# YujiaoShi/HighlyAccurate

Hardware: AMD Instinct MI355X
Metric: image-pairs/sec through N-iter LM pose loop, KITTI shapes (higher is better)
Workload: dtype bf16; 1 GPU; BASELINE configs[1]: LM_S2GP.forward(mode='test'), sat 512x512, grd 256x1024, VGG-16 two-branch, level 3, 5 LM iters x 3 levels, 3-DoF, random-init weights; pairs_per_gpu=32, global_batch=32, parallelism=batch-sharded x1, no collective

## Files before the change

### highlyaccurate_amd/csrc/common.h

```cpp
#pragma once
#include <hip/hip_runtime.h>
#include <atomic>
#include <stdarg.h>
#include <stdio.h>
#include "../../include/hla.h"

void hla_set_error(const char* fmt, ...);

enum { K_PACK = 0, K_CONV02, K_CONV_NT2, K_CONV_NT2_POOL, K_CONV_NT1, K_CONV_NT1_POOL, K_CONF, K_L2NORM,
       K_LM256, K_LM128, K_LM64, K_LM16, K_LMSOLVE, K_GRIDSAMPLE, K_LMBWD, K_WGRAD, K_ELEMWISE, K_LMREPAIR };
void hla_prof_begin(int id, double flops, double bytes, hipStream_t st);
void hla_prof_begin_dyn(int id, double flops, double bytes, hipStream_t st, const int* dev_live, int denom);
void hla_prof_end(hipStream_t st);
bool hla_prof_on();

#ifndef HLA_CONV_STAMPS
#define HLA_CONV_STAMPS 0
#endif
#if HLA_CONV_STAMPS
constexpr int HLA_STAMP_N = 8;
struct HlaStampCfg { unsigned long long* buf; int want; int counter; unsigned grid_x, grid_y; };
extern HlaStampCfg g_hla_stamp;
#endif

#define HLA_CHECK_HIP(expr)                                                              \
  do {                                                                                   \
    hipError_t _e = (expr);                                                              \
    if (_e != hipSuccess) {                                                              \
      hla_set_error("%s failed: %s (%s:%d)", #expr, hipGetErrorString(_e), __FILE__, __LINE__); \
      return HLA_ERR_HIP;                                                                \
    }                                                                                    \
  } while (0)

static inline bool hla_dtype_ok(int dtype) { return dtype == HLA_F32 || dtype == HLA_BF16 || dtype == HLA_F16 || dtype == HLA_F16X3; }

struct split32;
template <typename T> struct HlaType { using type = T; };
template <typename F> static inline auto hla_dispatch_dtype(int dtype, F&& f) {
  if (dtype == HLA_BF16) return f(HlaType<__bf16>{});
  if (dtype == HLA_F16) return f(HlaType<_Float16>{});
  if (dtype == HLA_F16X3) return f(HlaType<split32>{});
  return f(HlaType<float>{});
}

#define HLA_REQUIRE(cond, ...)      \
  do {                              \
    if (!(cond)) {                  \
      hla_set_error(__VA_ARGS__);   \
      return HLA_ERR_ARG;           \
    }                               \
  } while (0)

struct HlaPerDeviceOnce {
// ... 25 lines not shown
```

### highlyaccurate_amd/csrc/conv_kernels.h

```cpp
#pragma once
#include "common.h"
#include "conv_block_map.h"
#include <type_traits>

typedef __bf16 bf16;
typedef _Float16 f16;
using f32x16 = __attribute__((ext_vector_type(16))) float;
using bf16x8 = __attribute__((ext_vector_type(8))) __bf16;
using f16x8 = __attribute__((ext_vector_type(8))) _Float16;
using f16x4 = __attribute__((ext_vector_type(4))) _Float16;

struct split32 {
  float v;
  split32() = default;
  __host__ __device__ explicit split32(float f) : v(f) {}
  __host__ __device__ explicit operator float() const { return v; }
};
template <typename T> struct Prec { static constexpr bool SPLIT = false; static constexpr int CEPL = 16 / (int)sizeof(T); };
template <> struct Prec<split32> { static constexpr bool SPLIT = true; static constexpr int CEPL = 8; };

__device__ __host__ __forceinline__ float split_scale(unsigned amax_bits) {
  int E = (int)(amax_bits >> 23) & 0xff;
  E = E < 81 ? 81 : (E > 201 ? 201 : E);
  const unsigned bits = (unsigned)(127 + 141 - E) << 23;
// ... 166 lines not shown
  size_t wg0_x_plane;
  float* wg0_part;
#if HLA_CONV_STAMPS
  unsigned long long* stamps;
#endif
};
template <int NT> __host__ __device__ __forceinline__ int conv_cout_blocks(const ConvArgs& a) { return NT == 1 ? 1 : a.Cout / (64 * NT); }
#if HLA_CONV_STAMPS
#define HLA_STAMP(K) do { if (a.stamps) { const unsigned long long ts_ = __builtin_readcyclecounter(); \
    if ((threadIdx.x & 63) == 0) a.stamps[((size_t)blockIdx.x * 4 +(threadIdx.x >> 6)) * HLA_STAMP_N + (K)] = ts_; } } while (0)
#define HLA_STAMP_HWID() do { if (a.stamps && (threadIdx.x & 63) == 0) { \
    const unsigned long long hw_ = __builtin_amdgcn_s_getreg((31 << 11) | (0 << 6) | 4), xc_ = __builtin_amdgcn_s_getreg((31 << 11) | (0 << 6) | 20); \
    a.stamps[((size_t)blockIdx.x * 4 +(threadIdx.x >> 6)) * HLA_STAMP_N + 7] = hw_ | (xc_ << 32); } } while (0)
#else
#define HLA_STAMP(K) do {} while (0)
#define HLA_STAMP_HWID() do {} while (0)
#endif

struct ConvDyn {
  int n_live;
  int list;
  int src_bands;
  int add_bands;
};
struct PixBox { int y0, y1, x0, x1; };

constexpr int HWID = 34;
constexpr int SB = 64;
constexpr int PSTR = 64;
__device__ __forceinline__ int halo_key(int hx) { return (hx >> 2) & 3; }
__device__ __forceinline__ int halo_off(int pix, int hx, int slot) { return pix * PSTR + ((slot ^ halo_key(hx)) << 4); }
constexpr int HALO_TAP0 = 2, HALO_TAP1 = 6;
constexpr int HLA_CONV_DMA_TAP = 1;
struct FragOff { int o[3][2]; };
template <int SHAPE = SHAPE_32x32x16>
__device__ __forceinline__ FragOff frag_offsets(int lane, int row0) {
  FragOff f;
  if constexpr (SHAPE == SHAPE_16x16x32) {
    const int x = lane & 15, slot = lane >> 4;
#pragma unroll
    for (int kx = 0; kx < 3; ++kx)
#pragma unroll
      for (int p = 0; p < 2; ++p) f.o[kx][p] = halo_off(row0 * HWID + 16 * p + x + kx, 16 * p + x + kx, slot);
  } else {
    const int x = lane & 31, g = lane >> 5;
#pragma unroll
    for (int kx = 0; kx < 3; ++kx)
#pragma unroll
      for (int kg = 0; kg < 2; ++kg) f.o[kx][kg] = halo_off(row0 * HWID + x + kx, x + kx, g | (kg << 1));
  }
  return f;
}

__device__ __forceinline__ float lane_xor1(float v) {
  return __int_as_float(__builtin_amdgcn_update_dpp(0, __float_as_int(v), 0xB1, 0xF, 0xF, false));
}

template <typename E, int NT> struct RowStager {
  static constexpr int CW = NT * 32, PITCH = CW * (int)sizeof(E) + 16, CPP = CW * (int)sizeof(E) / 16;
  static __device__ __forceinline__ void put(char* stage, int px, int ch, float v0, float v1, float v2, float v3) {
    store4((E*)(stage + px * PITCH) + ch, v0, v1, v2, v3);
  }
  template <bool PLAIN = false, int GG = 2>
  static __device__ __forceinline__ float flush(const char* stage, E* dst, int npx, int npx_valid, int Cout, int lane,
                                                const E* mask = nullptr, const E* add = nullptr,
                                                int add_px_lo = 0, int add_px_hi = 1 << 30) {
// ... 450 lines not shown
        } else {
          const uint4 A = frag_kmajor<ET>(stage, PITCH, kk * KPX, 0, lane);
          ET e[EPV];
#pragma unroll
          for (int jj = 0; jj < EPV; ++jj) {
            const int k = sizeof(ET) == 2 ? 8 * g5 + jj : 2 * jj + g5;
            e[jj] = (ET)(j < 27 ? row[k] : (j == 27 ? 1.f : 0.f));
          }
          mma16<ET>(accw, A, __builtin_bit_cast(uint4, e));
        }
      }
      if (SPLIT) {
        const float ds = j == 27 ? 1.f / sG : 1.f / (sG * s_in);
#pragma unroll
        for (int r = 0; r < 16; ++r) accw[r] += tmp[r] * ds;
      }
    }
  }
  if (wm == 1) {
#pragma unroll
    for (int r = 0; r < 16; ++r) xr[(wn * 16 + r) * 64 + lane] = accw[r];
  }
  __syncthreads();
  if (wm == 0) {
    float* dst = a.wg0_part + (size_t)blockIdx.x * 64 * 32;
#pragma unroll
    for (int r = 0; r < 16; ++r) {
      const int co = cb + (r & 3) + 8 * (r >> 2) + 4 * g5;
      dst[co * 32 + j] = accw[r] + xr[(wn * 16 + r) * 64 + lane];
    }
  }
}

template <typename T, int MT, int NT, int WD, int PF = (NT == 1 ? 4 : 3)>
struct WeightRing {
  static constexpr int RS = WD + 1;
  uint4 wb[RS][2][NT];
  static constexpr int PFD = PF;
  uint4 pf[PFD + 1];
  const uint4* wq[NT];

  __device__ __forceinline__ void prime() {
#pragma unroll
    for (int d = 0; d < WD; ++d)
#pragma unroll
      for (int kg = 0; kg < 2; ++kg)
#pragma unroll
        for (int j = 0; j < NT; ++j) wb[d][kg][j] = wq[j][(d * 2 + kg) * 64];
  }
  __device__ __forceinline__ void next_stage() {
#pragma unroll
    for (int j = 0; j < NT; ++j) wq[j] += 18 * 64;
    if (9 % RS != 0) {
      uint4 tmp[WD][2][NT];
#pragma unroll
      for (int d = 0; d < WD; ++d)
#pragma unroll
        for (int kg = 0; kg < 2; ++kg)
#pragma unroll
          for (int j = 0; j < NT; ++j) tmp[d][kg][j] = wb[(9 + d) % RS][kg][j];
#pragma unroll
      for (int d = 0; d < WD; ++d)
#pragma unroll
        for (int kg = 0; kg < 2; ++kg)
#pragma unroll
          for (int j = 0; j < NT; ++j) wb[d][kg][j] = tmp[d][kg][j];
    }
  }
};

__device__ __forceinline__ void stagger_priority() {
  const unsigned slot = __builtin_amdgcn_s_getreg((3 << 11) | (0 << 6) | 4);
  if (slot & 1) __builtin_amdgcn_s_setprio(1);
}

template <typename T, int MT, int NT, int WD, int PF, int SHAPE = SHAPE_32x32x16, typename Mid>
__device__ __forceinline__ void stage_mma(typename AccMap<SHAPE>::Tile (&acc)[MT][NT], const char* cur, const FragOff& fo,
                                          WeightRing<T, MT, NT, WD, PF>& ring, Mid&& mid) {
  constexpr int RS = WD + 1;
#pragma unroll
  for (int tap = 0; tap < 9; ++tap) {
#pragma unroll
    for (int kg = 0; kg < 2; ++kg)
#pragma unroll
      for (int j = 0; j < NT; ++j) ring.wb[(tap + WD) % RS][kg][j] = ring.wq[j][((tap + WD) * 2 + kg) * 64];
    mid(tap);
    constexpr int FPT = MT * 2, DEPTH = PF;
    auto frag_ptr = [&](int f) {
      const int tp = tap + f / FPT, r = f % FPT;
      return cur + fo.o[tp % 3][r & 1] + (tp / 3 + (r >> 1)) * HWID * PSTR;
    };
    if (tap == 0) {
#pragma unroll
      for (int f = 0; f < DEPTH; ++f) ring.pf[f] = *(const uint4*)frag_ptr(f);
    }
    __builtin_amdgcn_sched_barrier(0);
#pragma unroll
    for (int f = 0; f < FPT; ++f) {
      const int slot = (tap * FPT + f) % (DEPTH + 1), nslot = (tap * FPT + f + DEPTH) % (DEPTH + 1);
      if (tap * FPT + f + DEPTH < 9 * FPT) ring.pf[nslot] = *(const uint4*)frag_ptr(f + DEPTH);
      const int i = f >> 1, kg = f & 1;
      if constexpr (Prec<T>::SPLIT) {
#pragma unroll
        for (int c = 0; c < (kg == 0 ? 2 : 1); ++c)
#pragma unroll
          for (int j = 0; j < NT; ++j) mma16<T>(acc[i][j], ring.wb[tap % RS][c][j], ring.pf[slot]);
      } else if constexpr (SHAPE == SHAPE_16x16x32) {
#pragma unroll
        for (int c = 0; c < 2; ++c)
#pragma unroll
          for (int j = 0; j < NT; ++j) mma32<T>(acc[i][j].t[2 * kg + c], ring.wb[tap % RS][c][j], ring.pf[slot]);
      } else {
#pragma unroll
        for (int j = 0; j < NT; ++j) mma16<T>(acc[i][j], ring.wb[tap % RS][kg][j], ring.pf[slot]);
      }
      __builtin_amdgcn_sched_barrier(0);
    }
  }
  ring.next_stage();
}

template <typename T, int MT, int NT, int WM, bool UNPOOL = false>
constexpr int conv3x3_lds_bytes() {
  constexpr int HP = (WM * MT + 2) * HWID, NP = (HP * 4 + 255) / 256;
  constexpr int buf = ((sizeof(T) == 2 && !UNPOOL && !Prec<T>::SPLIT) ? NP * 64 : HP) * PSTR;
  constexpr int stg = 32 * (RowStager<float, NT>::PITCH + (sizeof(T) == 2 ? RowStager<T, NT>::PITCH : 0));
  return 2 * buf > 4 * stg ? 2 * buf : 4 * stg;
}
template <typename T, int MT, int NT, int WM, int WN, bool POOL, int WD, bool UNPOOL = false, int SHAPE = SHAPE_32x32x16, bool XLDS = false>
__device__ __forceinline__ void conv3x3_body(const ConvArgs& a, const int blk, const int nblk) {
  static_assert(WM * WN == 4, "4 waves per block");
  static_assert(SHAPE == SHAPE_32x32x16 || (sizeof(T) == 2 && !UNPOOL), "16x16x32: bf16 / f16 forward kernels only");
  using M = AccMap<SHAPE>;
  constexpr int EPL = 16 / sizeof(T), KC = SB / sizeof(T);
  constexpr int TH = WM * MT, HPIX = (TH + 2) * HWID;
  constexpr int NPIECE = (HPIX * 4 + 255) / 256;
  constexpr bool DMA = sizeof(T) == 2 && !UNPOOL && !Prec<T>::SPLIT;
  constexpr int BUF = (DMA ? NPIECE * 64 : HPIX) * PSTR;
  constexpr int NHALF = (NPIECE + 1) / 2;
  constexpr int STG = 32 * (RowStager<float, NT>::PITCH + (sizeof(T) == 2 ? RowStager<T, NT>::PITCH : 0));
  constexpr int LDSB = 2 * BUF > 4 * STG ? 2 * BUF : 4 * STG;
  static_assert(LDSB == conv3x3_lds_bytes<T, MT, NT, WM, UNPOOL>(), "conv3x3_lds_bytes is what a launch with XLDS allocates");
  __shared__ __attribute__((aligned(16))) char lds_own[XLDS ? 16 : LDSB];
  extern __shared__ __attribute__((aligned(16))) char lds_dyn[];
  char* const lds = XLDS ? lds_dyn : lds_own;
  __shared__ float red[8];

  HLA_STAMP(0);
  HLA_STAMP_HWID();
  const int t = threadIdx.x, lane = t & 63, wv = __builtin_amdgcn_readfirstlane(t >> 6), wm = wv / WN, wn = wv % WN;
  const int sy0 = a.src_row_lo, sy1 = a.H;
  int tx, ty, b, cblk;
  const int gy = conv_cout_blocks<NT>(a);
  const int clo = a.col_begin * 32;
  struct { int lo0, lo1, lo2, hi0, hi1, hi2; } sb = {clo, clo, clo, a.W, a.W, a.W};
  if (a.dyn) {
    const ConvDyn& d = *(const ConvDyn*)(a.dyn + a.dyn_desc);
    const int nl = d.n_live, nlive = nl * a.B;
    if (blk >= nlive * gy) return;
    const ConvBlock m = conv_block_map(blk, nlive * gy, gy);
    const int bid = m.tile;
    cblk = __builtin_amdgcn_readfirstlane(m.cb);
    b = bid / nl;
    const int e = a.dyn[d.list + bid % nl];
// ... 142 lines not shown
                   HLA_DMA_LD(4, 7, 8) HLA_DMA_STEP HLA_DMA_LD(5, 7, 8) HLA_DMA_STEP HLA_DMA_LD(6, 7, 8) "s_mov_b32 m0, %0"             \
                   : "=&s"(keep) : "v"(O[0]), "v"(O[1]), "v"(O[2]), "v"(O[3]), "v"(O[4]), "v"(O[5]), "s"(rs), "s"(soff), "s"(dst)      \
                   : "memory", "scc")
      if (first) HLA_DMA6(off1); else HLA_DMA6(off2);
#undef HLA_DMA6
    } else if constexpr (NPIECE == 4) {
#define HLA_DMA4(O)                                                                                                                    \
      asm volatile(HLA_DMA_HEAD(7) HLA_DMA_LD(1, 5, 6) HLA_DMA_STEP HLA_DMA_LD(2, 5, 6) HLA_DMA_STEP HLA_DMA_LD(3, 5, 6) HLA_DMA_STEP    \
                   HLA_DMA_LD(4, 5, 6) "s_mov_b32 m0, %0"                                                                              \
                   : "=&s"(keep) : "v"(O[0]), "v"(O[1]), "v"(O[2]), "v"(O[3]), "s"(rs), "s"(soff), "s"(dst) : "memory", "scc")
      if (first) HLA_DMA4(off1); else HLA_DMA4(off2);
#undef HLA_DMA4
    }
#undef HLA_DMA_HEAD
#undef HLA_DMA_LD
#undef HLA_DMA_STEP
  };

  const int ntg0 = (cblk * WN + wn) * NT;
  typename M::Tile acc[MT][NT];
#pragma unroll
  for (int j = 0; j < NT; ++j)
#pragma unroll
    for (int q = 0; q < 4; ++q) {
      float4 b4 = make_float4(0.f, 0.f, 0.f, 0.f);
      if (sizeof(T) == 2 && a.bias) b4 = *(const float4*)(a.bias + (ntg0 + j) * 32 + M::ch(lane, q));
#pragma unroll
      for (int i = 0; i < MT; ++i) {
        M::set(acc[i][j], q, 0, b4.x); M::set(acc[i][j], q, 1, b4.y); M::set(acc[i][j], q, 2, b4.z); M::set(acc[i][j], q, 3, b4.w);
      }
    }

  const FragOff fo = frag_offsets<SHAPE>(lane, wm * MT);
  constexpr int PF = NT == 1 ? (UNPOOL && sizeof(T) == 2 ? 3 : 4) : 3;
  WeightRing<T, MT, NT, WD, PF> ring;
#pragma unroll
  for (int j = 0; j < NT; ++j) ring.wq[j] = a.wpk + (size_t)(ntg0 + j) * nstage * 18 * 64 + lane;

  uint4 st[NHALF];
  StageIds ids;
  ring.prime();
  if constexpr (DMA) {
    dma_stage(0, 0);
    asm volatile("s_waitcnt vmcnt(0)" ::: "memory");
  } else {
    uint4 st1[NHALF];
    StageIds ids1;
    load_stage(0, 0, st, ids);
    load_stage(0, 1, st1, ids1);
    write_stage(lds, 0, 0, st, ids);
    write_stage(lds, 0, 1, st1, ids1);
  }
  __syncthreads();
  HLA_STAMP(1);
  stagger_priority();

  for (int sg = 0; sg < nstage; ++sg) {
    const bool more = sg + 1 < nstage;
    char* nxt = lds + ((sg + 1) & 1) * BUF;
    stage_mma<T, MT, NT, WD, PF, SHAPE>(acc, lds + (sg & 1) * BUF, fo, ring, [&](int tap) __attribute__((always_inline)) {
      if constexpr (DMA) {
        if (tap == HLA_CONV_DMA_TAP && more) dma_stage(sg + 1, (sg + 1) & 1);
      } else {
        if (tap == HALO_TAP0 && more) load_stage(sg + 1, 0, st, ids);
        if (tap == HALO_TAP1 && more) { write_stage(nxt, sg + 1, 0, st, ids); load_stage(sg + 1, 1, st, ids); }
      }
    });
    if constexpr (DMA) {
      static_assert(!DMA || HLA_CONV_DMA_TAP <= 8 - WD, "the halo DMA must be issued before the next stage's weight fragments");
      if (more) asm volatile("s_waitcnt vmcnt(%0)" ::"n"(2 * NT * WD) : "memory");
    } else {
      if (more) write_stage(nxt, sg + 1, 1, st, ids);
    }
    if (sg == 0) HLA_STAMP(2);
    __syncthreads();
    if (sg == 0) HLA_STAMP(3);
  }
  HLA_STAMP(4);
  static_assert((LDSB / 4) % 16 == 0, "stager alignment");
  {
    char* stager = lds + wv * (LDSB / 4);
    const int mode = epilogue_mode(a);
    PixBox addb{a.add_row_lo, 1 << 30, 0, 1 << 30};
    if (a.dyn) {
      const ConvDyn& d = *(const ConvDyn*)(a.dyn + a.dyn_desc);
      if (d.add_bands >= 0) {
        const int band = (POOL ? y0 >> 1 : y0) >> 3;
        addb.x0 = a.dyn[d.add_bands + 2 * band];
        addb.x1 = a.dyn[d.add_bands + 2 * band + 1];
      }
    }
    constexpr bool RAW_SPECIAL = POOL || NT == 1;
    constexpr bool T16 = sizeof(T) == 2;
    if constexpr (UNPOOL && NT == 1 && MT == 4 && WN == 2) {
      if (mode == EPI_DGRAD_WG0) {
        conv_epilogue_wg0<T, MT>(acc, a, b, y0, x0, lds, dsc);
        HLA_STAMP(5);
        return;
      }
    }
    if (mode == EPI_ACT) conv_epilogue<T, MT, NT, POOL, EPI_ACT, false, LDSB / 4, SHAPE>(acc, a, b, y0 + wm * MT, x0, ntg0 * 32, red, stager, dsc, addb, nullptr, blk, nblk);
    else if (T16 && RAW_SPECIAL && a.raw16 && mode == EPI_ACT_RAW)
      conv_epilogue<T, MT, NT, POOL, (T16 && RAW_SPECIAL) ? EPI_ACT_RAW : EPI_GENERIC, T16 && RAW_SPECIAL, 0, SHAPE>(acc, a, b, y0 + wm * MT, x0, ntg0 * 32, red, stager, dsc, addb, nullptr, blk, nblk);
    else if (T16 && a.raw16 && mode == EPI_ACT_RAW_NOBIAS)
      conv_epilogue<T, MT, NT, POOL, T16 ? EPI_ACT_RAW_NOBIAS : EPI_GENERIC, T16, 0, SHAPE>(acc, a, b, y0 + wm * MT, x0, ntg0 * 32, red, stager, dsc, addb, nullptr, blk, nblk);
    else if (RAW_SPECIAL && mode == EPI_ACT_RAW) conv_epilogue<T, MT, NT, POOL, RAW_SPECIAL ? EPI_ACT_RAW : EPI_GENERIC, false, 0, SHAPE>(acc, a, b, y0 + wm * MT, x0, ntg0 * 32, red, stager, dsc, addb, nullptr, blk, nblk);
    else if (SHAPE == SHAPE_32x32x16 && mode == EPI_DGRAD)
      conv_epilogue<T, MT, NT, POOL, SHAPE == SHAPE_32x32x16 ? EPI_DGRAD : EPI_GENERIC, false, 0, SHAPE>(acc, a, b, y0 + wm * MT, x0, ntg0 * 32, red, stager, dsc, addb, nullptr, blk, nblk);
    else if ((RAW_SPECIAL || sizeof(T) == 2) && mode == EPI_ACT_RAW_NOBIAS)
      conv_epilogue<T, MT, NT, POOL, (RAW_SPECIAL || sizeof(T) == 2) ? EPI_ACT_RAW_NOBIAS : EPI_GENERIC, false, 0, SHAPE>(acc, a, b, y0 + wm * MT, x0, ntg0 * 32, red, stager, dsc, addb, nullptr, blk, nblk);
    else conv_epilogue<T, MT, NT, POOL, EPI_GENERIC, false, 0, SHAPE>(acc, a, b, y0 + wm * MT, x0, ntg0 * 32, red, stager, dsc, addb, nullptr, blk, nblk);
  }
  HLA_STAMP(5);
}
template <typename T, int MT, int NT, int WM, int WN, bool POOL, int WD, bool UNPOOL = false, int SHAPE = SHAPE_32x32x16>
__global__ __launch_bounds__(256, NT == 1 ? 3 : 2) void conv3x3_kernel(ConvArgs a) {
  conv3x3_body<T, MT, NT, WM, WN, POOL, WD, UNPOOL, SHAPE>(a, (int)blockIdx.x, (int)gridDim.x);
}

template <typename A> struct PairArgs { A s[2]; int n0; };
template <typename A>
__device__ __forceinline__ A kernarg_block(unsigned word_off) {
  static_assert(sizeof(A) % 4 == 0, "argument blocks are fetched as 32-bit words");
  typedef const __attribute__((address_space(4))) unsigned* kptr_t;
  const kptr_t kp = (kptr_t)__builtin_amdgcn_kernarg_segment_ptr() + word_off;
  unsigned w[sizeof(A) / 4];
#pragma unroll
  for (unsigned i = 0; i < sizeof(A) / 4; ++i) w[i] = kp[i];
  A a;
  __builtin_memcpy(&a, w, sizeof(A));
  return a;
}
template <typename A>
__device__ __forceinline__ A pair_segment_args(bool second) {
  static_assert(offsetof(PairArgs<A>, s) == 0, "the argument blocks lead the kernarg segment");
  return kernarg_block<A>(second ? sizeof(A) / 4 : 0);
}
template <typename P> __device__ __forceinline__ P* pair_global(P* p) {
  return (P*)(__attribute__((address_space(1))) P*)(unsigned long long)p;
}
__device__ __forceinline__ void pair_inference_args(ConvArgs& a) {
  a.src1 = pair_global(a.src1); a.src2 = pair_global(a.src2); a.wpk = pair_global(a.wpk); a.bias = pair_global(a.bias);
  a.out_act = pair_global(a.out_act); a.out_raw = pair_global(a.out_raw); a.sumsq = pair_global(a.sumsq);
  a.amax1 = pair_global(a.amax1); a.amax2 = pair_global(a.amax2); a.amax_out = pair_global(a.amax_out); a.wscale = pair_global(a.wscale);
  a.gate = nullptr; a.col_tiles = 0;
  a.dyn = nullptr; a.dyn_desc = 0; a.src_row_lo = 0; a.add_row_lo = 0; a.unpool_idx = nullptr; a.mask_act = nullptr; a.add_src = nullptr;
  a.idx_out = nullptr; a.pool_sum = 0; a.wg0_x = nullptr; a.wg0_x_plane = 0; a.wg0_part = nullptr;
#if HLA_CONV_STAMPS
  a.stamps = nullptr;
#endif
}
template <typename T, int MT, int NT, int WM, int WN, bool POOL, int WD, int SHAPE>
__global__ __launch_bounds__(256, NT == 1 ? 3 : 2) void conv3x3_pair_kernel(PairArgs<ConvArgs> p) {
  const int n0 = p.n0;
  const bool second = (int)blockIdx.x >= n0;
  ConvArgs a = pair_segment_args<ConvArgs>(second);
  pair_inference_args(a);
  conv3x3_body<T, MT, NT, WM, WN, POOL, WD, false, SHAPE>(a, second ? (int)blockIdx.x - n0 : (int)blockIdx.x,
                                                          second ? (int)gridDim.x - n0 : n0);
}

struct Conv02Args {
  const float* x;
  size_t x_plane;
  const uint4* w0;
  const float* b0;
  const uint4* w2;
  const float* b2;
  void* out_act;
  void* a0_out;
  unsigned char* idx_out;
  void* a2_out;
  int B, H, W, tiles_x, tiles_y;
  int row_begin;
  int col_begin;
  const int* gate;
  const float* wtail;
  unsigned* amax_out;
  unsigned* amax_a2_out;
  unsigned* amax_a0_out;
#if HLA_CONV_STAMPS
  unsigned long long* stamps;
#endif
};

template <typename T> constexpr int conv02_rounds() { return sizeof(T) == 4 ? 2 : 1; }
template <typename T> constexpr int conv02_lds_bytes() {
  return (64 * (int)sizeof(T) / SB) / conv02_rounds<T>() * (10 * HWID * PSTR) + 3 * 12 * 36 * 4;
}

template <typename T, int WD>
__device__ __forceinline__ void conv02_body(const Conv02Args& a0, const int blk) {
// ... 579 lines not shown
      else conv3x3_body<T, 4, 1, 2, 2, false, 2, false, S_NT1, true>(a, blk, nblk);
      __syncthreads();
    }
    fixup_layer_sync();
  }
  __shared__ double sh[4];
#pragma unroll
  for (int l = 0; l < 3; ++l) {
    inv_norm_row(pair_global(p.ss[l]), p.np[l], pair_global(p.inv[l]), b, sh);
    __syncthreads();
  }
}

struct ConvPlan { bool small; int gx, gy, kid; double flops, bytes; };
template <typename T, bool BWD>
static ConvPlan conv_plan(ConvArgs& a, bool pool) {
  const int txf = (a.W + 31) / 32;
  a.tiles_x = a.col_tiles ? a.col_tiles : txf - a.col_begin;
  if (a.col_begin + a.tiles_x > txf) a.tiles_x = txf - a.col_begin;
  a.tiles_y = (a.H - a.row_begin + 7) / 8;
  const int Wc = (a.col_begin + a.tiles_x == txf ? a.W : (a.col_begin + a.tiles_x) * 32) - a.col_begin * 32;
  const bool big = a.Cout >= 128;
  ConvPlan p{};
  p.gy = big ? a.Cout / 128 : 1;
  const size_t es = sizeof(T), P = (size_t)a.B * (a.H - a.row_begin) * Wc, Po = pool ? P / 4 : P;
  p.flops = 2.0 * 9.0 * (a.C1 + a.C2) * a.Cout * (double)P + (a.wg0_part ? 2.0 * 27 * 64 * (double)P : 0.0);
  p.bytes = (double)P * ((a.up1 ? a.C1 / 4.0 : a.C1) + a.C2) * es + (double)Po * a.Cout * ((a.out_act ? es : 0) + (a.out_raw ? 4 : 0));
  p.kid = big ? (pool ? K_CONV_NT2_POOL : K_CONV_NT2) : (pool ? K_CONV_NT1_POOL : K_CONV_NT1);
  p.small = !BWD && !a.dyn && !a.sumsq && !a.unpool_idx && a.tiles_x * a.tiles_y * a.B * p.gy < CONV_SMALL_GRID;
  if (p.small) a.tiles_y = (a.H - a.row_begin + 3) / 4;
  p.gx = a.tiles_x * a.tiles_y * a.B;
  return p;
}
template <typename T, int MT, int NT, bool POOL, int WD, bool UNPOOL, int SHAPE, bool PAIR>
static void conv_dispatch(hipStream_t st, const ConvArgs& a, const ConvPlan& p, const ConvArgs& a2, const ConvPlan& p2) {
  if constexpr (PAIR) {
    static_assert(!UNPOOL, "two-segment launches: forward inference forms only");
    PairArgs<ConvArgs> pa{{a, a2}, p.gx * p.gy};
    hipLaunchKernelGGL((conv3x3_pair_kernel<T, MT, NT, 2, 2, POOL, WD, SHAPE>), dim3((p.gx + p2.gx) * p.gy), dim3(256), 0, st, pa);
  } else {
    hipLaunchKernelGGL((conv3x3_kernel<T, MT, NT, 2, 2, POOL, WD, UNPOOL, SHAPE>), dim3(p.gx * p.gy), dim3(256), 0, st, a);
  }
}
template <typename T, bool BWD, bool PAIR>
static bool launch_conv_impl(hipStream_t st, ConvArgs a, ConvArgs a2, bool pool) {
  if (a.unpool_idx && !(BWD && !pool)) {
    hla_set_error("launch_conv: an un-pooled source needs the UNPOOL kernel (backward, no pooling epilogue)");
    return false;
  }
  const ConvPlan p = conv_plan<T, BWD>(a, pool);
  ConvPlan p2{};
  if constexpr (PAIR) {
    p2 = conv_plan<T, BWD>(a2, pool);
    auto infer = [](const ConvArgs& c) {
      return !c.dyn && !c.src_row_lo && !c.add_row_lo && !c.unpool_idx && !c.mask_act && !c.add_src && !c.idx_out && !c.pool_sum && !c.wg0_part;
    };
    if (BWD || !infer(a) || !infer(a2) || p2.small != p.small || p2.gy != p.gy || a2.Cout != a.Cout) {
      hla_set_error("launch_conv: the two segments of a paired launch do not take the same kernel");
      return false;
    }
  }
#if HLA_CONV_STAMPS
  a.stamps = a2.stamps = nullptr;
  if (!PAIR && g_hla_stamp.buf && g_hla_stamp.counter++ == g_hla_stamp.want) {
    a.stamps = g_hla_stamp.buf;
    g_hla_stamp.grid_x = a.tiles_x * ((a.H - a.row_begin + 7) / 8) * a.B; g_hla_stamp.grid_y = p.gy;
  }
#endif
  const bool big = a.Cout >= 128;
  hla_prof_begin_dyn(p.kid, p.flops + p2.flops, p.bytes + p2.bytes, st, a.dyn ? a.dyn + a.dyn_desc : nullptr, a.tiles_x * a.tiles_y);
  constexpr int S_NT2 = conv_shape<T, BWD>(CONV_CLASS_NT2), S_NT2P = conv_shape<T, BWD>(CONV_CLASS_NT2_POOL),
                S_NT1 = conv_shape<T, BWD>(CONV_CLASS_NT1);
  constexpr bool UNP = BWD && !PAIR;
  if (p.small) {
    if constexpr (!BWD) {
      if (big) {
        if (pool) conv_dispatch<T, 2, 2, true, 1, false, S_NT2P, PAIR>(st, a, p, a2, p2);
        else conv_dispatch<T, 2, 2, false, 1, false, S_NT2, PAIR>(st, a, p, a2, p2);
      } else {
        if (pool) conv_dispatch<T, 2, 1, true, 2, false, S_NT1, PAIR>(st, a, p, a2, p2);
        else conv_dispatch<T, 2, 1, false, 2, false, S_NT1, PAIR>(st, a, p, a2, p2);
      }
    }
    hla_prof_end(st);
    return true;
  }
  if (big) {
    if (pool) conv_dispatch<T, 4, 2, true, 1, false, S_NT2P, PAIR>(st, a, p, a2, p2);
    else if (UNP && a.unpool_idx) conv_dispatch<T, 4, 2, false, 1, UNP, S_NT2, PAIR>(st, a, p, a2, p2);
    else conv_dispatch<T, 4, 2, false, 1, false, S_NT2, PAIR>(st, a, p, a2, p2);
  } else {
    if (pool) conv_dispatch<T, 4, 1, true, 2, false, S_NT1, PAIR>(st, a, p, a2, p2);
    else if (UNP && a.unpool_idx) conv_dispatch<T, 4, 1, false, 2, UNP, S_NT1, PAIR>(st, a, p, a2, p2);
    else conv_dispatch<T, 4, 1, false, 2, false, S_NT1, PAIR>(st, a, p, a2, p2);
  }
  hla_prof_end(st);
  return true;
}
template <typename T, bool BWD = false>
static bool launch_conv(hipStream_t st, const ConvArgs& a, bool pool) { return launch_conv_impl<T, BWD, false>(st, a, ConvArgs{}, pool); }
template <typename T>
static bool launch_conv_pair(hipStream_t st, const ConvArgs& a, const ConvArgs& a2, bool pool) {
  return launch_conv_impl<T, false, true>(st, a, a2, pool);
}
```

### highlyaccurate_amd/csrc/vgg.hip

```cpp
#include "conv_kernels.h"
#include "vgg_layers.h"
#include <type_traits>

template <typename T>
void vgg_pack_all(const hla_vgg_params* prm, char* packed, int dtype, hipStream_t st) {
  constexpr bool SPLIT = Prec<T>::SPLIT;
  std::conditional_t<SPLIT, SplitPackTable, PackTable> tb{};
  if constexpr (!SPLIT) tb.b0 = prm->b[0];
  int n = 0;
  for (int l = 0; l < kAllLayers; ++l) {
    if (l >= kPackedLayers && !prm->w[l]) continue;
    tb.w[n] = prm->w[l]; tb.off[n] = packed_offset(l, dtype); tb.cout[n] = kLayers[l].cout; tb.cin[n] = kLayers[l].cin;
    tb.first[n] = l == 0 ? 1 : 0;
    if constexpr (SPLIT) tb.slot[n] = l;
    else tb.shape[n] = l >= 2 ? conv_shape<T, false>(conv_class(kLayers[l].cout, vgg_layer_pools(l))) : SHAPE_32x32x16;
    ++n;
  }
  if constexpr (!SPLIT) {
    hla_prof_begin(K_PACK, 0, (double)packed_offset(kAllLayers, dtype) * (1.0 + 4.0 / sizeof(T)), st);
    hipLaunchKernelGGL((pack_weights_multi_kernel<T>), dim3(256, n), dim3(256), 0, st, tb, packed);
  } else {
    float* tail = (float*)(packed + packed_offset(kAllLayers, dtype));
    unsigned* scratch = (unsigned*)tail + 32;
    (void)hipMemsetAsync(tail, 0, kPackTailBytes, st);
// ... 209 lines not shown
    return hipFuncSetAttribute((const void*)vgg_fixup_loop<T>, hipFuncAttributeMaxDynamicSharedMemorySize, lds_bytes);
  }));
  hipLaunchKernelGGL((vgg_fixup_loop<T>), dim3(c.B), dim3(256), lds_bytes, c.st, fa);
  HLA_CHECK_HIP(hipGetLastError());
  return HLA_OK;
}

constexpr int HLA_PAIR_FALLBACK = -1000;
template <typename T>
int vgg_forward_pair_t(const VggFwdCall c[2]) {
  constexpr bool SPLIT = Prec<T>::SPLIT;
  hipStream_t st = c[0].st;
  VggConvSet S[2];
  for (int k = 0; k < 2; ++k) vgg_build_convs<T>(c[k], false, S[k]);
  for (int l = 2; l < kAllLayers; ++l) {
    if (S[0].used[l] != S[1].used[l]) return HLA_PAIR_FALLBACK;
    if (!S[0].used[l]) continue;
    ConvArgs a0 = S[0].conv[l], a1 = S[1].conv[l];
    if (conv_plan<T, false>(a0, S[0].pool[l]).small != conv_plan<T, false>(a1, S[1].pool[l]).small) return HLA_PAIR_FALLBACK;
  }
  if (SPLIT)
    for (int k = 0; k < 2; ++k)
      HLA_CHECK_HIP(hipMemsetAsync(c[k].ws + c[k].pl.amax, 0, (size_t)kAmaxSlots * c[k].B * sizeof(unsigned), st));
  if (const int rc = launch_conv02<T>(st, S[0].c02, &S[1].c02)) return rc;
  bool launch_ok = true;
  for (int l = 2; l < kAllLayers; ++l)
    if (S[0].used[l] && !launch_conv_pair<T>(st, S[0].conv[l], S[1].conv[l], S[0].pool[l])) launch_ok = false;
  const VggFwdCall* nets[2] = {&c[0], &c[1]};
  if (const int rc = vgg_norms(2, nets, S, 3)) return rc;
  HLA_CHECK_HIP(hipGetLastError());
  return launch_ok ? HLA_OK : HLA_ERR_ARG;
}

#if HLA_TU_DTYPE >= 0
template void vgg_pack_all<TuT>(const hla_vgg_params* prm, char* packed, int dtype, hipStream_t st);
template int vgg_forward_t<TuT>(const VggFwdCall& c);
template int vgg_forward_pair_t<TuT>(const VggFwdCall c[2]);
#if HLA_TU_DTYPE == 1 || HLA_TU_DTYPE == 2
template int vgg_fixup_t<TuT>(const VggFwdCall& c);
#endif
#else
#define HLA_EXTERN_T(T) \
  extern template void vgg_pack_all<T>(const hla_vgg_params* prm, char* packed, int dtype, hipStream_t st); \
  extern template int vgg_forward_t<T>(const VggFwdCall& c); \
  extern template int vgg_forward_pair_t<T>(const VggFwdCall c[2]);
HLA_EXTERN_T(float) HLA_EXTERN_T(bf16) HLA_EXTERN_T(f16) HLA_EXTERN_T(split32)
extern template int vgg_fixup_t<bf16>(const VggFwdCall& c);
extern template int vgg_fixup_t<f16>(const VggFwdCall& c);

extern "C" size_t hla_vgg_packed_weight_bytes(int dtype) {
  return packed_offset(kAllLayers, dtype) + (dtype == HLA_F16X3 ? kPackTailBytes : 0);
}

extern "C" int hla_vgg_pack_weights(const hla_vgg_params* params, void* packed, int dtype, hla_stream_t stream) {
  HLA_REQUIRE(params && packed, "hla_vgg_pack_weights: null argument");
  HLA_REQUIRE(hla_dtype_ok(dtype), "hla_vgg_pack_weights: bad dtype %d", dtype);
  HLA_REQUIRE(params->w[0] && params->b[0], "hla_vgg_pack_weights: conv0's weight and bias are required (the bias is packed with it)");
  hla_dispatch_dtype(dtype, [&](auto t) { vgg_pack_all<typename decltype(t)::type>(params, (char*)packed, dtype, (hipStream_t)stream); });
  HLA_CHECK_HIP(hipGetLastError());
  return HLA_OK;
}

extern "C" size_t hla_vgg_workspace_bytes(int B, int H, int W, int level, int dtype) {
  VggPlan p;
  vgg_plan(B, H, W, dtype, true, &p, level == 4);
  return p.total;
}

extern "C" size_t hla_vgg_workspace_bytes_flags(int B, int H, int W, int level, int dtype, int flags) {
  VggPlan p;
  vgg_plan(B, H, W, dtype, true, &p, level == 4, (flags & HLA_VGG_FOLD_DECODER) != 0);
  return p.total;
}

static inline int vgg_first_col32(int first_col32, int level, int dtype, int flags) {
  const bool ok = level == 3 && dtype != HLA_F16X3 && (flags & HLA_VGG_DEFER_NORM) &&
                  !(flags & (HLA_VGG_SAVE_FOR_BACKWARD | HLA_VGG_FOLD_DECODER | HLA_VGG_WANT_CONF));
  return ok ? first_col32 : 0;
}

static int vgg_forward_check(VggFwdCall& c, bool silent) {
// ... 100 lines not shown
```

Before: 6267 pairs/s.

## Load conv weight fragments with hand-counted async loads alongside the halo DMA

For bf16/fp16 forward convolutions, weight fragments now come from inline-asm global_load_dwordx4 into a ring with explicit s_waitcnt vmcnt counts. These waits are coordinated with the outstanding halo DMA requests, so the compiler no longer inserts conservative waits that stall the MMA loop. NT=2 kernels get a deeper weight ring (WD 2 instead of 1) with a shallower activation prefetch. MT=2 async kernels are also asked for higher occupancy through launch_bounds. A debug single-layer conv entry point and extra timing stamps are added as well; counting vmcnt by hand is fragile and raises register pressure.

```diff
diff --git a/highlyaccurate_amd/csrc/common.h b/highlyaccurate_amd/csrc/common.h
--- a/highlyaccurate_amd/csrc/common.h
+++ b/highlyaccurate_amd/csrc/common.h
@@ -18,7 +18,7 @@
 #define HLA_CONV_STAMPS 0
 #endif
 #if HLA_CONV_STAMPS
-constexpr int HLA_STAMP_N = 8;
+constexpr int HLA_STAMP_N = 16;
 struct HlaStampCfg { unsigned long long* buf; int want; int counter; unsigned grid_x, grid_y; };
 extern HlaStampCfg g_hla_stamp;
 #endif
diff --git a/highlyaccurate_amd/csrc/conv_kernels.h b/highlyaccurate_amd/csrc/conv_kernels.h
--- a/highlyaccurate_amd/csrc/conv_kernels.h
+++ b/highlyaccurate_amd/csrc/conv_kernels.h
@@ -222,6 +222,9 @@
 __device__ __forceinline__ int halo_off(int pix, int hx, int slot) { return pix * PSTR + ((slot ^ halo_key(hx)) << 4); }
 constexpr int HALO_TAP0 = 2, HALO_TAP1 = 6;
 constexpr int HLA_CONV_DMA_TAP = 1;
+#ifndef HLA_CONV_ASYNC_RING
+#define HLA_CONV_ASYNC_RING 1
+#endif
 struct FragOff { int o[3][2]; };
 template <int SHAPE = SHAPE_32x32x16>
 __device__ __forceinline__ FragOff frag_offsets(int lane, int row0) {
@@ -738,15 +741,51 @@
   }
 }
 
-template <typename T, int MT, int NT, int WD, int PF = (NT == 1 ? 4 : 3)>
+typedef unsigned u32x4 __attribute__((ext_vector_type(4)));
+template <typename T, int MT, int NT, int WD, int PF = (NT == 1 ? 4 : 3), bool ASYNC = false>
 struct WeightRing {
   static constexpr int RS = WD + 1;
+  static_assert(!ASYNC || 9 % RS == 0, "fragments in flight across the stage boundary must keep their ring slot");
+  static_assert(!ASYNC || NT <= 2, "wait() names 2 * NT fragments");
   uint4 wb[RS][2][NT];
+  u32x4 wa[RS][2][NT];
+  const char* ws[NT];
+  unsigned lane16;
+  __device__ __forceinline__ uint4 frag(int slot, int c, int j) const {
+    if constexpr (ASYNC) return __builtin_bit_cast(uint4, wa[slot][c][j]);
+    else return wb[slot][c][j];
+  }
+  __device__ __forceinline__ void request(int slot, int tapi) {
+#pragma unroll
+    for (int kg = 0; kg < 2; ++kg)
+#pragma unroll
+      for (int j = 0; j < NT; ++j) {
+        if constexpr (ASYNC) {
+          const char* p = ws[j] + (tapi * 2 + kg) * 1024;
+          asm volatile("global_load_dwordx4 %0, %1, %2" : "=v"(wa[slot][kg][j]) : "v"(lane16), "s"(p));
+        } else {
+          wb[slot][kg][j] = wq[j][(tapi * 2 + kg) * 64];
+        }
+      }
+  }
+  template <int N, int N0 = N> __device__ __forceinline__ void wait(int slot, bool alt = false) {
+    if (N0 != N && alt) asm volatile("s_waitcnt vmcnt(%0)" ::"n"(N0));
+    else asm volatile("s_waitcnt vmcnt(%0)" ::"n"(N));
+    if constexpr (NT == 2)
+      asm volatile("" : "+v"(wa[slot][0][0]), "+v"(wa[slot][0][1]), "+v"(wa[slot][1][0]), "+v"(wa[slot][1][1]));
+    else
+      asm volatile("" : "+v"(wa[slot][0][0]), "+v"(wa[slot][1][0]));
+  }
   static constexpr int PFD = PF;
   uint4 pf[PFD + 1];
   const uint4* wq[NT];
 
   __device__ __forceinline__ void prime() {
+    if constexpr (ASYNC) {
+#pragma unroll
+      for (int d = 0; d < WD; ++d) request(d, d);
+      return;
+    }
 #pragma unroll
     for (int d = 0; d < WD; ++d)
 #pragma unroll
@@ -755,6 +794,11 @@
         for (int j = 0; j < NT; ++j) wb[d][kg][j] = wq[j][(d * 2 + kg) * 64];
   }
   __device__ __forceinline__ void next_stage() {
+    if constexpr (ASYNC) {
+#pragma unroll
+      for (int j = 0; j < NT; ++j) ws[j] += 18 * 1024;
+      return;
+    }
 #pragma unroll
     for (int j = 0; j < NT; ++j) wq[j] += 18 * 64;
     if (9 % RS != 0) {
@@ -780,17 +824,37 @@
   if (slot & 1) __builtin_amdgcn_s_setprio(1);
 }
 
-template <typename T, int MT, int NT, int WD, int PF, int SHAPE = SHAPE_32x32x16, typename Mid>
+#if HLA_CONV_STAMPS
+struct StageStamps { bool on; unsigned long long t0, w[5]; };
+#endif
+template <typename T, int MT, int NT, int WD, int PF, int SHAPE = SHAPE_32x32x16, int DMAN = 0, bool ASYNC = false, typename Mid>
 __device__ __forceinline__ void stage_mma(typename AccMap<SHAPE>::Tile (&acc)[MT][NT], const char* cur, const FragOff& fo,
-                                          WeightRing<T, MT, NT, WD, PF>& ring, Mid&& mid) {
+                                          WeightRing<T, MT, NT, WD, PF, ASYNC>& ring, Mid&& mid, bool more = false
+#if HLA_CONV_STAMPS
+                                          , StageStamps* ss = nullptr
+#endif
+                                          ) {
   constexpr int RS = WD + 1;
+  static_assert(ASYNC == (DMAN > 0), "the hand-counted ring belongs to the DMA halo loader");
 #pragma unroll
   for (int tap = 0; tap < 9; ++tap) {
-#pragma unroll
-    for (int kg = 0; kg < 2; ++kg)
-#pragma unroll
-      for (int j = 0; j < NT; ++j) ring.wb[(tap + WD) % RS][kg][j] = ring.wq[j][((tap + WD) * 2 + kg) * 64];
+    if constexpr (ASYNC) {
+      ring.request((tap + WD) % RS, tap + WD);
+    } else {
+#pragma unroll
+      for (int kg = 0; kg < 2; ++kg)
+#pragma unroll
+        for (int j = 0; j < NT; ++j) ring.wb[(tap + WD) % RS][kg][j] = ring.wq[j][((tap + WD) * 2 + kg) * 64];
+    }
     mid(tap);
+#if HLA_CONV_STAMPS
+    const bool stamped = ss && ss->on && ((tap >= HLA_CONV_DMA_TAP && tap <= HLA_CONV_DMA_TAP + 3) || tap == 8);
+    if (stamped) ss->t0 = __builtin_readcyclecounter();
+#endif
+    if constexpr (ASYNC) {
+      if (tap >= HLA_CONV_DMA_TAP && tap <= HLA_CONV_DMA_TAP + WD) ring.template wait<2 * NT * WD, 2 * NT * WD + DMAN>(tap % RS, more);
+      else ring.template wait<2 * NT * WD>(tap % RS);
+    }
     constexpr int FPT = MT * 2, DEPTH = PF;
     auto frag_ptr = [&](int f) {
       const int tp = tap + f / FPT, r = f % FPT;
@@ -810,17 +874,20 @@
 #pragma unroll
         for (int c = 0; c < (kg == 0 ? 2 : 1); ++c)
 #pragma unroll
-          for (int j = 0; j < NT; ++j) mma16<T>(acc[i][j], ring.wb[tap % RS][c][j], ring.pf[slot]);
+          for (int j = 0; j < NT; ++j) mma16<T>(acc[i][j], ring.frag(tap % RS, c, j), ring.pf[slot]);
       } else if constexpr (SHAPE == SHAPE_16x16x32) {
 #pragma unroll
         for (int c = 0; c < 2; ++c)
 #pragma unroll
-          for (int j = 0; j < NT; ++j) mma32<T>(acc[i][j].t[2 * kg + c], ring.wb[tap % RS][c][j], ring.pf[slot]);
+          for (int j = 0; j < NT; ++j) mma32<T>(acc[i][j].t[2 * kg + c], ring.frag(tap % RS, c, j), ring.pf[slot]);
       } else {
 #pragma unroll
-        for (int j = 0; j < NT; ++j) mma16<T>(acc[i][j], ring.wb[tap % RS][kg][j], ring.pf[slot]);
+        for (int j = 0; j < NT; ++j) mma16<T>(acc[i][j], ring.frag(tap % RS, kg, j), ring.pf[slot]);
       }
       __builtin_amdgcn_sched_barrier(0);
+#if HLA_CONV_STAMPS
+      if (f == 0 && stamped) ss->w[tap == 8 && HLA_CONV_DMA_TAP + 3 < 8 ? 4 : tap - HLA_CONV_DMA_TAP] += __builtin_readcyclecounter() - ss->t0;
+#endif
     }
   }
   ring.next_stage();
@@ -833,9 +900,11 @@
   constexpr int stg = 32 * (RowStager<float, NT>::PITCH + (sizeof(T) == 2 ? RowStager<T, NT>::PITCH : 0));
   return 2 * buf > 4 * stg ? 2 * buf : 4 * stg;
 }
-template <typename T, int MT, int NT, int WM, int WN, bool POOL, int WD, bool UNPOOL = false, int SHAPE = SHAPE_32x32x16, bool XLDS = false>
+template <typename T, int MT, int NT, int WM, int WN, bool POOL, int WD, bool UNPOOL = false, int SHAPE = SHAPE_32x32x16, bool XLDS = false,
+          bool WRA = false>
 __device__ __forceinline__ void conv3x3_body(const ConvArgs& a, const int blk, const int nblk) {
   static_assert(WM * WN == 4, "4 waves per block");
+  static_assert(!WRA || (sizeof(T) == 2 && !UNPOOL), "the hand-counted weight ring counts the DMA halo loader's requests");
   static_assert(SHAPE == SHAPE_32x32x16 || (sizeof(T) == 2 && !UNPOOL), "16x16x32: bf16 / f16 forward kernels only");
   using M = AccMap<SHAPE>;
   constexpr int EPL = 16 / sizeof(T), KC = SB / sizeof(T);
@@ -1044,10 +1113,14 @@
     }
 
   const FragOff fo = frag_offsets<SHAPE>(lane, wm * MT);
-  constexpr int PF = NT == 1 ? (UNPOOL && sizeof(T) == 2 ? 3 : 4) : 3;
-  WeightRing<T, MT, NT, WD, PF> ring;
-#pragma unroll
-  for (int j = 0; j < NT; ++j) ring.wq[j] = a.wpk + (size_t)(ntg0 + j) * nstage * 18 * 64 + lane;
+  constexpr int PF = NT == 1 ? (UNPOOL && sizeof(T) == 2 ? 3 : 4) : (WRA ? 2 : 3);
+  WeightRing<T, MT, NT, WD, PF, WRA> ring;
+#pragma unroll
+  for (int j = 0; j < NT; ++j) {
+    if constexpr (WRA) ring.ws[j] = (const char*)(a.wpk + (size_t)(ntg0 + j) * nstage * 18 * 64);
+    else ring.wq[j] = a.wpk + (size_t)(ntg0 + j) * nstage * 18 * 64 + lane;
+  }
+  if constexpr (WRA) ring.lane16 = lane * 16;
 
   uint4 st[NHALF];
   StageIds ids;
@@ -1055,6 +1128,10 @@
   if constexpr (DMA) {
     dma_stage(0, 0);
     asm volatile("s_waitcnt vmcnt(0)" ::: "memory");
+    if constexpr (WRA) {
+#pragma unroll
+      for (int d = 0; d < WD; ++d) ring.template wait<0>(d);
+    }
   } else {
     uint4 st1[NHALF];
     StageIds ids1;
@@ -1067,27 +1144,60 @@
   HLA_STAMP(1);
   stagger_priority();
 
+#if HLA_CONV_STAMPS
+  StageStamps ss = {false, 0, {0, 0, 0, 0, 0}};
+  unsigned long long ss_req = 0, ss_bar = 0, ss_stage = 0, ss_n = 0;
+#endif
   for (int sg = 0; sg < nstage; ++sg) {
     const bool more = sg + 1 < nstage;
     char* nxt = lds + ((sg + 1) & 1) * BUF;
-    stage_mma<T, MT, NT, WD, PF, SHAPE>(acc, lds + (sg & 1) * BUF, fo, ring, [&](int tap) __attribute__((always_inline)) {
+#if HLA_CONV_STAMPS
+    ss.on = a.stamps && sg >= 1 && more;
+    const unsigned long long ts_stage = __builtin_readcyclecounter();
+#endif
+    stage_mma<T, MT, NT, WD, PF, SHAPE, WRA ? NPIECE : 0>(acc, lds + (sg & 1) * BUF, fo, ring, [&](int tap) __attribute__((always_inline)) {
       if constexpr (DMA) {
-        if (tap == HLA_CONV_DMA_TAP && more) dma_stage(sg + 1, (sg + 1) & 1);
+        if (tap == HLA_CONV_DMA_TAP && more) {
+#if HLA_CONV_STAMPS
+          const unsigned long long ts_req = __builtin_readcyclecounter();
+#endif
+          dma_stage(sg + 1, (sg + 1) & 1);
+#if HLA_CONV_STAMPS
+          if (ss.on) ss_req += __builtin_readcyclecounter() - ts_req;
+#endif
+        }
       } else {
         if (tap == HALO_TAP0 && more) load_stage(sg + 1, 0, st, ids);
         if (tap == HALO_TAP1 && more) { write_stage(nxt, sg + 1, 0, st, ids); load_stage(sg + 1, 1, st, ids); }
       }
-    });
+    }, more
+#if HLA_CONV_STAMPS
+    , &ss
+#endif
+    );
+#if HLA_CONV_STAMPS
+    const unsigned long long ts_end = __builtin_readcyclecounter();
+#endif
     if constexpr (DMA) {
       static_assert(!DMA || HLA_CONV_DMA_TAP <= 8 - WD, "the halo DMA must be issued before the next stage's weight fragments");
       if (more) asm volatile("s_waitcnt vmcnt(%0)" ::"n"(2 * NT * WD) : "memory");
+      else if constexpr (WRA) asm volatile("s_waitcnt vmcnt(0)" ::: "memory");
     } else {
       if (more) write_stage(nxt, sg + 1, 1, st, ids);
     }
     if (sg == 0) HLA_STAMP(2);
     __syncthreads();
     if (sg == 0) HLA_STAMP(3);
-  }
+#if HLA_CONV_STAMPS
+    if (ss.on) { const unsigned long long te = __builtin_readcyclecounter(); ss_bar += te - ts_end; ss_stage += te - ts_stage; ++ss_n; }
+#endif
+  }
+#if HLA_CONV_STAMPS
+  if (a.stamps && (threadIdx.x & 63) == 0) {
+    unsigned long long* o = a.stamps + ((size_t)blockIdx.x * 4 + (threadIdx.x >> 6)) * HLA_STAMP_N;
+    o[6] = ss_n; o[8] = ss_req; o[9] = ss.w[0]; o[10] = ss.w[1]; o[11] = ss.w[2]; o[12] = ss.w[3]; o[13] = ss.w[4]; o[14] = ss_bar; o[15] = ss_stage;
+  }
+#endif
   HLA_STAMP(4);
   static_assert((LDSB / 4) % 16 == 0, "stager alignment");
   {
@@ -1125,9 +1235,9 @@
   }
   HLA_STAMP(5);
 }
-template <typename T, int MT, int NT, int WM, int WN, bool POOL, int WD, bool UNPOOL = false, int SHAPE = SHAPE_32x32x16>
-__global__ __launch_bounds__(256, NT == 1 ? 3 : 2) void conv3x3_kernel(ConvArgs a) {
-  conv3x3_body<T, MT, NT, WM, WN, POOL, WD, UNPOOL, SHAPE>(a, (int)blockIdx.x, (int)gridDim.x);
+template <typename T, int MT, int NT, int WM, int WN, bool POOL, int WD, bool UNPOOL = false, int SHAPE = SHAPE_32x32x16, bool WRA = false>
+__global__ __launch_bounds__(256, (NT == 1 || (WRA && MT == 2)) ? 3 : 2) void conv3x3_kernel(ConvArgs a) {
+  conv3x3_body<T, MT, NT, WM, WN, POOL, WD, UNPOOL, SHAPE, false, WRA>(a, (int)blockIdx.x, (int)gridDim.x);
 }
 
 template <typename A> struct PairArgs { A s[2]; int n0; };
@@ -1162,14 +1272,14 @@
   a.stamps = nullptr;
 #endif
 }
-template <typename T, int MT, int NT, int WM, int WN, bool POOL, int WD, int SHAPE>
-__global__ __launch_bounds__(256, NT == 1 ? 3 : 2) void conv3x3_pair_kernel(PairArgs<ConvArgs> p) {
+template <typename T, int MT, int NT, int WM, int WN, bool POOL, int WD, int SHAPE, bool WRA>
+__global__ __launch_bounds__(256, (NT == 1 || (WRA && MT == 2)) ? 3 : 2) void conv3x3_pair_kernel(PairArgs<ConvArgs> p) {
   const int n0 = p.n0;
   const bool second = (int)blockIdx.x >= n0;
   ConvArgs a = pair_segment_args<ConvArgs>(second);
   pair_inference_args(a);
-  conv3x3_body<T, MT, NT, WM, WN, POOL, WD, false, SHAPE>(a, second ? (int)blockIdx.x - n0 : (int)blockIdx.x,
-                                                          second ? (int)gridDim.x - n0 : n0);
+  conv3x3_body<T, MT, NT, WM, WN, POOL, WD, false, SHAPE, false, WRA>(a, second ? (int)blockIdx.x - n0 : (int)blockIdx.x,
+                                                                      second ? (int)gridDim.x - n0 : n0);
 }
 
 struct Conv02Args {
@@ -1815,14 +1925,14 @@
   p.gx = a.tiles_x * a.tiles_y * a.B;
   return p;
 }
-template <typename T, int MT, int NT, bool POOL, int WD, bool UNPOOL, int SHAPE, bool PAIR>
+template <typename T, int MT, int NT, bool POOL, int WD, bool UNPOOL, int SHAPE, bool PAIR, bool WRA = false>
 static void conv_dispatch(hipStream_t st, const ConvArgs& a, const ConvPlan& p, const ConvArgs& a2, const ConvPlan& p2) {
   if constexpr (PAIR) {
     static_assert(!UNPOOL, "two-segment launches: forward inference forms only");
     PairArgs<ConvArgs> pa{{a, a2}, p.gx * p.gy};
-    hipLaunchKernelGGL((conv3x3_pair_kernel<T, MT, NT, 2, 2, POOL, WD, SHAPE>), dim3((p.gx + p2.gx) * p.gy), dim3(256), 0, st, pa);
+    hipLaunchKernelGGL((conv3x3_pair_kernel<T, MT, NT, 2, 2, POOL, WD, SHAPE, WRA>), dim3((p.gx + p2.gx) * p.gy), dim3(256), 0, st, pa);
   } else {
-    hipLaunchKernelGGL((conv3x3_kernel<T, MT, NT, 2, 2, POOL, WD, UNPOOL, SHAPE>), dim3(p.gx * p.gy), dim3(256), 0, st, a);
+    hipLaunchKernelGGL((conv3x3_kernel<T, MT, NT, 2, 2, POOL, WD, UNPOOL, SHAPE, WRA>), dim3(p.gx * p.gy), dim3(256), 0, st, a);
   }
 }
 template <typename T, bool BWD, bool PAIR>
@@ -1855,27 +1965,29 @@
   constexpr int S_NT2 = conv_shape<T, BWD>(CONV_CLASS_NT2), S_NT2P = conv_shape<T, BWD>(CONV_CLASS_NT2_POOL),
                 S_NT1 = conv_shape<T, BWD>(CONV_CLASS_NT1);
   constexpr bool UNP = BWD && !PAIR;
+  constexpr bool WRA = HLA_CONV_ASYNC_RING && !BWD && sizeof(T) == 2;
+  constexpr int WD2 = WRA ? 2 : 1;
   if (p.small) {
     if constexpr (!BWD) {
       if (big) {
-        if (pool) conv_dispatch<T, 2, 2, true, 1, false, S_NT2P, PAIR>(st, a, p, a2, p2);
-        else conv_dispatch<T, 2, 2, false, 1, false, S_NT2, PAIR>(st, a, p, a2, p2);
+        if (pool) conv_dispatch<T, 2, 2, true, WD2, false, S_NT2P, PAIR, WRA>(st, a, p, a2, p2);
+        else conv_dispatch<T, 2, 2, false, WD2, false, S_NT2, PAIR, WRA>(st, a, p, a2, p2);
       } else {
-        if (pool) conv_dispatch<T, 2, 1, true, 2, false, S_NT1, PAIR>(st, a, p, a2, p2);
-        else conv_dispatch<T, 2, 1, false, 2, false, S_NT1, PAIR>(st, a, p, a2, p2);
+        if (pool) conv_dispatch<T, 2, 1, true, 2, false, S_NT1, PAIR, WRA>(st, a, p, a2, p2);
+        else conv_dispatch<T, 2, 1, false, 2, false, S_NT1, PAIR, WRA>(st, a, p, a2, p2);
       }
     }
     hla_prof_end(st);
     return true;
   }
   if (big) {
-    if (pool) conv_dispatch<T, 4, 2, true, 1, false, S_NT2P, PAIR>(st, a, p, a2, p2);
-    else if (UNP && a.unpool_idx) conv_dispatch<T, 4, 2, false, 1, UNP, S_NT2, PAIR>(st, a, p, a2, p2);
-    else conv_dispatch<T, 4, 2, false, 1, false, S_NT2, PAIR>(st, a, p, a2, p2);
+    if (pool) conv_dispatch<T, 4, 2, true, WD2, false, S_NT2P, PAIR, WRA>(st, a, p, a2, p2);
+    else if (UNP && a.unpool_idx) { if constexpr (UNP) conv_dispatch<T, 4, 2, false, 1, true, S_NT2, PAIR>(st, a, p, a2, p2); }
+    else conv_dispatch<T, 4, 2, false, WD2, false, S_NT2, PAIR, WRA>(st, a, p, a2, p2);
   } else {
-    if (pool) conv_dispatch<T, 4, 1, true, 2, false, S_NT1, PAIR>(st, a, p, a2, p2);
-    else if (UNP && a.unpool_idx) conv_dispatch<T, 4, 1, false, 2, UNP, S_NT1, PAIR>(st, a, p, a2, p2);
-    else conv_dispatch<T, 4, 1, false, 2, false, S_NT1, PAIR>(st, a, p, a2, p2);
+    if (pool) conv_dispatch<T, 4, 1, true, 2, false, S_NT1, PAIR, WRA>(st, a, p, a2, p2);
+    else if (UNP && a.unpool_idx) { if constexpr (UNP) conv_dispatch<T, 4, 1, false, 2, true, S_NT1, PAIR>(st, a, p, a2, p2); }
+    else conv_dispatch<T, 4, 1, false, 2, false, S_NT1, PAIR, WRA>(st, a, p, a2, p2);
   }
   hla_prof_end(st);
   return true;
diff --git a/highlyaccurate_amd/csrc/vgg.hip b/highlyaccurate_amd/csrc/vgg.hip
--- a/highlyaccurate_amd/csrc/vgg.hip
+++ b/highlyaccurate_amd/csrc/vgg.hip
@@ -265,7 +265,37 @@
   return launch_ok ? HLA_OK : HLA_ERR_ARG;
 }
 
+struct HlaConvLayerSeg {
+  const void* src;
+  const float* w;
+  void* wpk;
+  void* out;
+  float* raw;
+  double* sumsq;
+  int H, W;
+};
+struct HlaConvLayerCall { int B, Cin, Cout, pool, nseg; HlaConvLayerSeg seg[2]; hipStream_t st; };
+template <typename T>
+int vgg_conv_layer_t(const HlaConvLayerCall& c) {
+  ConvArgs a[2] = {};
+  for (int k = 0; k < c.nseg; ++k) {
+    const HlaConvLayerSeg& s = c.seg[k];
+    PackTable tb{};
+    tb.w[0] = s.w; tb.off[0] = 0; tb.cout[0] = c.Cout; tb.cin[0] = c.Cin; tb.first[0] = 0;
+    tb.shape[0] = conv_shape<T, false>(conv_class(c.Cout, c.pool != 0));
+    hipLaunchKernelGGL((pack_weights_multi_kernel<T>), dim3(64, 1), dim3(256), 0, c.st, tb, (char*)s.wpk);
+    a[k].src1 = s.src; a[k].wpk = (const uint4*)s.wpk; a[k].out_act = s.out; a[k].out_raw = s.raw; a[k].sumsq = s.raw ? s.sumsq : nullptr;
+    a[k].C1 = c.Cin; a[k].B = c.B; a[k].H = s.H; a[k].W = s.W; a[k].Cout = c.Cout; a[k].relu_act = 1;
+  }
+  const bool ok = c.nseg == 2 ? launch_conv_pair<T>(c.st, a[0], a[1], c.pool != 0) : launch_conv<T>(c.st, a[0], c.pool != 0);
+  HLA_CHECK_HIP(hipGetLastError());
+  return ok ? HLA_OK : HLA_ERR_ARG;
+}
+
 #if HLA_TU_DTYPE >= 0
+#if HLA_TU_DTYPE == 1 || HLA_TU_DTYPE == 2
+template int vgg_conv_layer_t<TuT>(const HlaConvLayerCall& c);
+#endif
 template void vgg_pack_all<TuT>(const hla_vgg_params* prm, char* packed, int dtype, hipStream_t st);
 template int vgg_forward_t<TuT>(const VggFwdCall& c);
 template int vgg_forward_pair_t<TuT>(const VggFwdCall c[2]);
@@ -280,6 +310,23 @@
 HLA_EXTERN_T(float) HLA_EXTERN_T(bf16) HLA_EXTERN_T(f16) HLA_EXTERN_T(split32)
 extern template int vgg_fixup_t<bf16>(const VggFwdCall& c);
 extern template int vgg_fixup_t<f16>(const VggFwdCall& c);
+extern template int vgg_conv_layer_t<bf16>(const HlaConvLayerCall& c);
+extern template int vgg_conv_layer_t<f16>(const HlaConvLayerCall& c);
+
+extern "C" int hla_debug_conv_layer(int dtype, int B, int Cin, int Cout, int pool, const void* seg, int nseg, hla_stream_t stream) {
+  HLA_REQUIRE(seg && (nseg == 1 || nseg == 2), "hla_debug_conv_layer: one or two segments");
+  HLA_REQUIRE(dtype == HLA_BF16 || dtype == HLA_F16, "hla_debug_conv_layer: bf16 / fp16 only");
+  HLA_REQUIRE(B > 0 && Cin >= 32 && Cin % 32 == 0 && (Cout == 64 || (Cout >= 128 && Cout % 128 == 0)),
+              "hla_debug_conv_layer: Cin a multiple of 32, Cout 64 or a multiple of 128 (got %d, %d)", Cin, Cout);
+  HlaConvLayerCall c{B, Cin, Cout, pool, nseg, {}, (hipStream_t)stream};
+  for (int k = 0; k < nseg; ++k) {
+    c.seg[k] = ((const HlaConvLayerSeg*)seg)[k];
+    const HlaConvLayerSeg& s = c.seg[k];
+    HLA_REQUIRE(s.src && s.w && s.wpk && s.out && s.H > 0 && s.W > 0 && (!pool || (s.H % 2 == 0 && s.W % 2 == 0)) && (!s.raw || s.sumsq),
+                "hla_debug_conv_layer: segment %d: null argument, odd size under the pool, or raw without sumsq", k);
+  }
+  return dtype == HLA_BF16 ? vgg_conv_layer_t<bf16>(c) : vgg_conv_layer_t<f16>(c);
+}
 
 extern "C" size_t hla_vgg_packed_weight_bytes(int dtype) {
   return packed_offset(kAllLayers, dtype) + (dtype == HLA_F16X3 ? kPackTailBytes : 0);
```

Result: faster. 6387 pairs/s (median of 6 runs) (+1.9%).
